# aim-uofa/GenPercept

Hardware: NVIDIA H100
Metric: images/sec at 768x768 depth (higher is better)
Workload: dtype f16

## Files before the change

genpercept_b200/csrc/builder.cu:

```cuda
#include <algorithm>
#include <cmath>
#include <cstring>

#include <cstdlib>

#include "engine.h"
#include "fattn.h"
#include "fattn512.h"

namespace gp {

constexpr size_t kFusedAttnMinBytes = size_t(2) << 30;

size_t Arena::alloc(size_t bytes) {
  bytes = (bytes + 1023) & ~size_t(1023);
  if (bytes == 0) bytes = 1024;
  for (size_t i = 0; i < blks_.size(); ++i) {
    if (blks_[i].free && blks_[i].size >= bytes) {
      if (blks_[i].size > bytes) {
        Blk rest{blks_[i].off + bytes, blks_[i].size - bytes, true};
        blks_[i].size = bytes;
        blks_.insert(blks_.begin() + i + 1, rest);
      }
      blks_[i].free = false;
// ... 130 lines not shown
  *mt = ts.mt;
}

static void check_cuda(cudaError_t e, const std::string& what) {
  if (e != cudaSuccess) throw GpError(GP_ERR_CUDA, what + ": " + cudaGetErrorString(e));
}
static void finalize_or_throw(IgemmParams* p, const std::string& name) {
  const char* err = igemm_finalize(p);
  if (err) throw GpError(GP_ERR_INVALID, name + ": " + err);
}

static bool gn_fusable(const ConvArgs& a, bool split) {
  const char* on = std::getenv("GP_GN_FUSE");
  const bool off = on == nullptr || on[0] == '0';
  if (off || split || a.mode != 0 || a.ks != 3 || a.srcs.size() != 1 || a.sc.size() > 1) return false;
  const T4& s = a.srcs[0];
  if ((s.W % 128) || (s.C % 64) || (!a.sc.empty() && (a.sc[0].C % 64))) return false;
  const int Cout = a.cout_valid > 0 ? a.cout_valid : a.out.C;
  if (!a.out_f32 && (Cout != a.out.C || (Cout % 64))) return false;
  if (a.flags & IG_GEGLU) return false;
  return true;
}

void Builder::conv(const std::string& name, const ConvArgs& a) {
  GP_REQUIRE(!a.srcs.empty() && a.w != nullptr, name + ": bad conv args");
  const bool gn_fused = a.gn != nullptr && gn_fusable(a, split_);
  if (a.gn != nullptr && !gn_fused) {
    int ctot = 0;
    for (auto& s : a.srcs) ctot += s.C;
    T4 tmp = alloc(a.srcs[0].N, a.srcs[0].H, a.srcs[0].W, ctot);
// ... 23 lines not shown
  for (auto& s : a.sc) bytes += (double)s.bytes();
  if (a.res1) bytes += (double)a.res1->bytes();
  if (a.res2) bytes += (double)a.res2->bytes();
  if (!a.out_f32) GP_REQUIRE(a.out.N == N && a.out.H == Ho && a.out.W == Wo, name + ": output shape mismatch");
  const bool tokens_mode = (a.ks == 1 && a.mode == 0 && a.sc.empty() && a.srcs.size() == 1 && !a.out_f32);
  const long long work_px = tokens_mode ? (long long)N * H * W
                                        : (long long)(a.mode == 3 ? W : Wo) * (a.mode == 3 ? H : Ho) * N * (a.mode == 3 ? 4 : 1);
  int bn_pre = choose_bn(Cout, a.force_bn);
  int mt_pre = (bn_pre <= 64 && work_px >= 256LL * num_sms) ? 2 : 1;
  if (!a.force_bn && !(a.flags & IG_GEGLU) && !gn_fused) {
    const double k_elems = flops / (2.0 * N * Ho * Wo * (double)Cout) * (a.mode == 3 ? 4.0 / 9.0 : 1.0);
    tile_shape_for(Cout, k_elems, tokens_mode, N * (a.mode == 3 ? 4 : 1), (a.mode == 3) ? W : Wo, (a.mode == 3) ? H : Ho, num_sms,
                   &bn_pre, &mt_pre);
  }
  const bool staged = !a.out_f32 && !(a.flags & IG_GEGLU) && Cout == a.out.C && (Cout % 64) == 0 && (bn_pre % 64) == 0;
  const bool patch_eligible = gn_fused || (staged && a.mode == 0 && a.ks == 3 && a.srcs.size() == 1 && a.sc.empty() &&
                                           work_px >= 128LL * num_sms && (W % 128) == 0 && !split_);
  if (patch_eligible) {
    bn_pre = (bn_pre == 128 && mt_pre == 1 && staged) ? 128 : 64;
    mt_pre = 1;
  }
  bool emit_stats = a.want_stats && staged && Cout <= 512 && !split_;
  if (emit_stats && tokens_mode && ((long long)H * W) % (128 * mt_pre) != 0) emit_stats = false;
  size_t stats_off = 0;
  const size_t stats_bytes = (size_t)N * num_sms * Cout * 2 * sizeof(float);
  if (emit_stats) {
    GP_REQUIRE(stats.find(a.out.off) == stats.end(), name + ": output already has statistics");
    stats_off = arena_.alloc(stats_bytes);
    stats[a.out.off] = StatsInfo{stats_off, num_sms, Cout};
  }
  if (measuring_) return;

  IgemmParams p;
  std::memset(&p, 0, sizeof(p));
  p.flags = a.flags | (bf16_ ? IG_BF16 : 0) | (a.out_f32 ? IG_OUT_F32_NCHW : 0);
  p.bias = a.w->bias;
  p.res1 = a.res1 ? ptr(*a.res1) : nullptr;
  p.res2 = a.res2 ? ptr(*a.res2) : nullptr;
  p.out = a.out_f32 ? (void*)a.out_f32 : ptr(a.out);
  p.Cout = Cout;
  p.BN = bn_pre;
  p.Z1 = 1; p.Z0 = 1;
  p.out_sy = p.out_sx = 1;
  const bool tokens = tokens_mode;
// ... 161 lines not shown
    p.tmPatch2 = p.tmPatch;
    if (!a.sc.empty()) {
      const T4& x = a.sc[0];
      p.kc_sc = ceil_div(x.C, 64);
      check_cuda(make_tmap_a(&p.tmPatch2, ptr(x), x.C, W, H, N, x.C, (long long)W * x.C, (long long)H * W * x.C,
                             p.TW + 2, p.TH + 2, bf16_), name + ": tmap patch (shortcut)");
    }
    if (gn_fused) {
      p.gn_ss = gn_ss;
      p.gn_C = s0.C;
      p.gn_silu = a.gn_silu ? 1 : 0;
    }
  }
  if (emit_stats) {
    p.stats = reinterpret_cast<float*>(raw_ptr(stats_off));
    p.stats_slots = num_sms;
    p.stats_hw = tokens ? H * W : 0;
  }
  finalize_or_throw(&p, name);
  GP_REQUIRE(p.MT == mt_pre && p.BN == bn_pre, name + ": tile pre-selection disagrees with the plan");
  const int ncls = p.cls_from_z0 ? p.Z0 : 1;
  for (int c = 0; c < ncls; ++c)
    GP_REQUIRE(p.nkb[c] * 64 == a.w->ktot, name + ": packed K (" + std::to_string(a.w->ktot) + ") != planned K (" +
                                              std::to_string(p.nkb[c] * 64) + ")");
  GP_REQUIRE(a.w->rows >= Cout || a.w->rows == Cout, name + ": packed rows < Cout");
  if (emit_stats) {
    float* sp = p.stats;
    push(name, 2, flops, bytes, [p, sp, stats_bytes](cudaStream_t s) {
      cudaError_t e = cudaMemsetAsync(sp, 0, stats_bytes, s);
      if (e != cudaSuccess) return e;
      return igemm_launch(p, s);
// ... 416 lines not shown
```

genpercept_b200/csrc/igemm.cu:

```cuda
#include "igemm.h"

#include <cstring>

#include "igemm_common.cuh"
#include "launch.h"

namespace gp {

namespace {

template <bool BF16, int BN, int MB>
__device__ __forceinline__ void tap_consumer(const IgemmParams& p, uint8_t* smem, int stage_bytes, int a_bytes, float* accs,
                                             uint64_t* full_bar, uint64_t* empty_bar, uint64_t* tfull_bar, uint64_t* tempty_bar,
                                             int wc, int lane) {
  float d[MB][BN / 2];
  int stage = 0;
  uint32_t phase = 0, acc_phase = 0;
  for (int tile = blockIdx.x; tile < p.total_tiles; tile += gridDim.x) {
    const TileCoord t = decode_tile(p, tile);
    const int cls = p.cls_from_z0 ? t.z0 : 0;
    const int nkb = p.nkb[cls] * p.npass;
    int held = -1;
    for (int kb = 0; kb < nkb; ++kb) {
      mbar_wait(&full_bar[stage], phase, 3);
// ... 72 lines not shown
      mbar_init(&full_bar[i], 2);
      mbar_init(&empty_bar[i], 4);
    }
    mbar_init(tfull_bar, 128);
    mbar_init(tempty_bar, kEpiWarps * 32);
    for (int i = 0; i < kEpiWarps; ++i) mbar_init(&res_bar[i], 1);
    fence_barrier_init();
  }
  __syncthreads();

  if (warp < 8) {
    setmaxnreg_inc<kWorkerRegs>();
    if (warp >= kConsumerWarp0) {
      run_tap_consumer<BF16>(p, smem, stage_bytes, a_bytes, accs, full_bar, empty_bar, tfull_bar, tempty_bar, warp - kConsumerWarp0, lane);
    } else {
      if (p.tma_store) run_epilogue_staged<BF16, false>(p, stg_base, sacc, sbias, tfull_bar, tempty_bar, res_bar, accs, warp, lane);
      else run_epilogue_direct<BF16>(p, sbias, tfull_bar, tempty_bar, accs, warp, lane);
    }
    return;
  }
  setmaxnreg_dec<kProducerRegs>();

  if (warp == 8) {
    const bool leader = elect_one();
    int stage = 0;
    uint32_t phase = 0;
    for (int tile = blockIdx.x; tile < p.total_tiles; tile += gridDim.x) {
      const TileCoord t = decode_tile(p, tile);
      const int cls = p.cls_from_z0 ? t.z0 : 0;
      const int a_n = t.z1 * p.a_n_z1 + t.z0 * p.a_n_z0;
      const int a_k0 = t.z0 * p.a_k_z0;
// ... 120 lines not shown
  p->tiles_x = (p->gridW + p->TW - 1) / p->TW;
  p->tiles_y = (p->gridH + p->TH - 1) / p->TH;
  p->n_tiles_n = (p->Cout + p->BN - 1) / p->BN;
  const int ncls = p->cls_from_z0 ? p->Z0 : 1;
  if (ncls > kMaxClasses) return "too many classes";
  for (int c = 0; c < ncls; ++c) {
    if (p->nseg[c] < 1 || p->nseg[c] > kMaxSegs) return "bad segment count";
    int n = 0;
    for (int s = 0; s < p->nseg[c]; ++s) n += p->seg[c][s].nchunks;
    p->nkb[c] = n;
    if (n < 1) return "empty K loop";
  }
  long long total = (long long)p->n_tiles_n * p->tiles_x * p->tiles_y * p->Z0 * p->Z1;
  if (total > 0x7fffffffLL) return "too many tiles";
  p->total_tiles = (int)total;
  const int stats_bytes = p->stats ? 4 * p->Cout * 2 * (int)sizeof(float) : 0;
  if (p->tma_store && ((p->Cout % 64) || (p->BN % 64) || (p->flags & (IG_OUT_F32_NCHW | IG_GEGLU)) || p->out_z0 != 0))
    return "staged epilogue needs Cout % 64 == 0, BN % 64 == 0, plain 16-bit NHWC output, no GEGLU";
  if (p->stats && (!p->tma_store || p->Cout > 512)) return "statistics need the staged epilogue and Cout <= 512";
  p->acc_half = (p->patch && p->BN == 128) ? 1 : 0;
  if (p->acc_half && (!p->tma_store || p->MT != 1))
    return "patch mode at BN = 128 needs the staged epilogue and MT = 1";
  p->acc_pitch = p->acc_half ? 64 : (p->BN + 31) & ~31;
  const int fixed = (p->tma_store ? kEpiWarps * 4096 * (p->out_lo ? 2 : 1) : 0) + acc_tile_bytes(*p) + 3072 + stats_bytes;
  const int ring_unit = p->patch ? p->BN * 128 : kABytes * p->MT + p->BN * 128;
  if (p->patch) {
    if (p->TW != 128 || p->TH != p->MT || p->Z0 != 1 || p->Z1 < 1 || p->nseg[0] != 9 + (p->kc_sc > 0 ? 1 : 0) || p->kc_count < 1 ||
        p->nkb[0] != 9 * p->kc_count + p->kc_sc || p->npass != 1 || p->gridW % 128 || p->gridH % p->TH)
      return "patch mode needs TW = 128, TH = MT, full tiles and a single-source 3x3 tap table (+ shortcut chunks)";
    if (p->gn_ss && p->gn_C != p->kc_count * 64) return "patch mode: GroupNorm channels must equal the source's";
    p->a_slot_bytes = ((p->TW + 2) * (p->TH + 2) * 128 + 1023) & ~1023;
  }
  const int avail = kMaxSmem - 1024 - fixed - (p->patch ? 2 * p->a_slot_bytes : 0);
  int st = avail / ring_unit;
  p->bias_slots = kBiasSlots;
  p->bias_all = 0;
  if (p->n_tiles_n > 1 && p->n_tiles_n * p->BN + 32 <= 4096) {
    const int extra = (p->n_tiles_n * p->BN + 32 - kBiasSlots) * (int)sizeof(float);
    if ((avail - extra) / ring_unit == st) {
      p->bias_all = 1;
      p->bias_slots = p->n_tiles_n * p->BN + 32;
    }
  }
  if (st > 8) st = 8;
  if (st < 2) return "tile too large for shared memory";
  p->stages = st;
  return nullptr;
// ... 9 lines not shown
    cudaError_t e = cudaFuncSetAttribute(igemm_kernel<false>, cudaFuncAttributeMaxDynamicSharedMemorySize, kMaxSmem);
    if (e != cudaSuccess) return e;
    e = cudaFuncSetAttribute(igemm_kernel<true>, cudaFuncAttributeMaxDynamicSharedMemorySize, kMaxSmem);
    if (e != cudaSuccess) return e;
    cudaDeviceGetAttribute(&sms[dev], cudaDevAttrMultiProcessorCount, dev);
    attr_set[dev] = true;
  }
  g_num_sms = sms[dev];
  return cudaSuccess;
}

cudaError_t igemm_launch(const IgemmParams& p, cudaStream_t stream) {
  cudaError_t ie = igemm_init();
  if (ie != cudaSuccess) return ie;
  if (p.total_tiles <= 0) return cudaSuccess;
  if (p.stats && p.stats_slots < (p.total_tiles < g_num_sms ? p.total_tiles : g_num_sms)) return cudaErrorInvalidValue;
  const int grid = p.total_tiles < g_num_sms ? p.total_tiles : g_num_sms;
  const size_t smem = kMaxSmem;
  if (p.patch) return igemm_patch_launch(p, grid, stream);
  if (p.flags & IG_BF16) {
    launch(igemm_kernel<true>, grid, kRoleThreads, smem, stream, p);
  } else {
    launch(igemm_kernel<false>, grid, kRoleThreads, smem, stream, p);
  }
  return cudaGetLastError();
}

}
```

genpercept_b200/csrc/igemm.h:

```cpp
#pragma once
#include <cuda.h>
#include <cuda_runtime.h>
#include <stdint.h>

namespace gp {

constexpr int kMaxSegs = 20;
constexpr int kMaxClasses = 4;
constexpr int kBM = 128;
constexpr int kBK = 64;

struct IgemmSeg {
  int8_t map;
  int8_t dy, dx;
  uint16_t nchunks;
};

enum IgemmFlags : int {
  IG_RELU = 1,
  IG_OUT_F32_NCHW = 2,
  IG_AFFINE_CLAMP01 = 4,
  IG_BF16 = 8,
  IG_GEGLU = 16,
};
// ... 30 lines not shown
  const float* bias;
  const void* res1;
  const void* res2;
  int flags;
  int stages;
  int total_tiles;
  float* stats;
  int stats_slots;
  int stats_hw;
  int tma_store;
  CUtensorMap tmOut[kMaxClasses];
  int res_tma;
  int bias_slots;
  int bias_all;
  int acc_pitch;
  int acc_half;
  CUtensorMap tmRes[kMaxClasses];
  int patch;
  int kc_count;
  int kc_sc;
  int a_slot_bytes;
  CUtensorMap tmPatch;
  CUtensorMap tmPatch2;
  const float* gn_ss;
  int gn_C;
  int gn_silu;
};

cudaError_t igemm_patch_launch(const IgemmParams& p, int grid, cudaStream_t stream);

cudaError_t make_tmap_a(CUtensorMap* m, const void* base, int C, int W, int H, int N, long long sW,
// ... 8 lines not shown
```

genpercept_b200/csrc/igemm_common.cuh:

```cuda
#pragma once
#include <cuda_bf16.h>
#include <cuda_fp16.h>

#include "igemm.h"
#include "ptx.cuh"

namespace gp {
namespace {

constexpr int kABytes = kBM * kBK * 2;
constexpr int kMaxSmem = 227 * 1024;
constexpr int kEpiWarps = 4;
constexpr int kConsumerWarp0 = 4;
constexpr int kRoleThreads = 384;
constexpr int kProducerRegs = 40;
constexpr int kWorkerRegs = 232;
static_assert(128 * kProducerRegs + 256 * kWorkerRegs <= 65536, "register file of one SM");

struct TileCoord {
  int n_tile, tx, ty, z0, z1;
};

__device__ __forceinline__ TileCoord decode_tile(const IgemmParams& p, int tile) {
  TileCoord t;
// ... 63 lines not shown
  for (int q = 0; q < N / 4; ++q) {
    const float4 v = *reinterpret_cast<const float4*>(rp + (acc_chunk((c >> 2) + q, row) << 2));
    r[4 * q] = __float_as_uint(v.x); r[4 * q + 1] = __float_as_uint(v.y);
    r[4 * q + 2] = __float_as_uint(v.z); r[4 * q + 3] = __float_as_uint(v.w);
  }
}

template <int BN, bool BF16>
__device__ __forceinline__ void wgmma_ss(float (&d)[BN / 2], uint64_t a, uint64_t b, uint32_t acc) {
  if constexpr (BN == 16) wgmma_ss_n16<BF16>(d, a, b, acc);
  else if constexpr (BN == 32) wgmma_ss_n32<BF16>(d, a, b, acc);
  else if constexpr (BN == 64) wgmma_ss_n64<BF16>(d, a, b, acc);
  else wgmma_ss_n128<BF16>(d, a, b, acc);
}

template <int BN, int MB, int J0 = 0, int NJ = BN / 8>
__device__ __forceinline__ void acc_store(float* accs, int pitch, float (&d)[MB][BN / 2], int wc, int lane) {
#pragma unroll
  for (int mb = 0; mb < MB; ++mb) {
    reg_fence(d[mb]);
#pragma unroll
    for (int j = J0; j < J0 + NJ; ++j)
#pragma unroll
      for (int hh = 0; hh < 2; ++hh) {
        const int row = 64 * mb + 16 * wc + (lane >> 2) + 8 * hh, col = 8 * (j - J0) + 2 * (lane & 3);
        *reinterpret_cast<float2*>(accs + (size_t)row * pitch + (acc_chunk(col >> 2, row) << 2) + (col & 3)) =
            make_float2(d[mb][4 * j + 2 * hh], d[mb][4 * j + 2 * hh + 1]);
      }
  }
}

__device__ __forceinline__ float gelu_erf(float g) {
  const float z = fabsf(g) * 0.70710678118654752f;
  float t;
  asm("rcp.approx.ftz.f32 %0, %1;" : "=f"(t) : "f"(fmaf(0.3275911f, z, 1.f)));
  float e;
  asm("ex2.approx.ftz.f32 %0, %1;" : "=f"(e) : "f"(z * z * -1.4426950408889634f));
  float q = fmaf(1.061405429f, t, -1.453152027f);
  q = fmaf(q, t, 1.421413741f);
  q = fmaf(q, t, -0.284496736f);
// ... 25 lines not shown
}

template <bool BF16, bool SPLIT, int RES>
__device__ __forceinline__ void epilogue_staged(const IgemmParams& p, uint8_t* stg_base, float* sacc, float* sbias, uint64_t* tfull_bar,
                                                uint64_t* tempty_bar, uint64_t* res_bar, const float* accs, int warp, int lane) {
  const int wq = warp;
  uint8_t* stg = stg_base + warp * 4096;
  const uint32_t stg_addr = smem_u32(stg);
  const uint32_t my_row = stg_addr + lane * 128;
  constexpr bool split = SPLIT;
  const uint32_t my_row_lo = my_row + kEpiWarps * 4096;
  const int sw = lane & 7;
  uint32_t acc_phase = 0, res_phase = 0;
  const bool relu = (p.flags & IG_RELU) != 0;
  const bool do_stats = p.stats != nullptr;
  const bool halves = p.acc_half != 0;
  const int etid = threadIdx.x;
  int cur_img = -1;
  int cur_nt = -1;
  auto flush_stats = [&](int img) {
    epi_sync();
    float* dst = p.stats + ((long long)img * p.stats_slots + blockIdx.x) * p.Cout * 2;
    for (int i = etid; i < 2 * p.Cout; i += kEpiWarps * 32) {
      const float tot = (sacc[i] + sacc[2 * p.Cout + i]) + (sacc[4 * p.Cout + i] + sacc[6 * p.Cout + i]);
      dst[i] = tot;
      sacc[i] = 0.f; sacc[2 * p.Cout + i] = 0.f; sacc[4 * p.Cout + i] = 0.f; sacc[6 * p.Cout + i] = 0.f;
    }
    epi_sync();
  };
  if (do_stats) {
    for (int i = etid; i < 8 * p.Cout; i += kEpiWarps * 32) sacc[i] = 0.f;
// ... 26 lines not shown
        if (cur_img >= 0) flush_stats(cur_img);
        cur_img = img;
      }
    }
    for (int h = 0; h < p.MT; ++h) {
      const int r0 = h * 128 + wq * 32;
      const int row = r0 + lane;
      const int ti = row >> p.tw_shift, tj = row & (p.TW - 1);
      const int gy = t.ty * p.TH + ti, gx = t.tx * p.TW + tj;
      const bool valid = gy < p.gridH && gx < p.gridW;
      const int oy = gy * p.out_sy + p.cls_py[cls], ox = gx * p.out_sx + p.cls_px[cls];
      const long long pix_off = t.z1 * p.out_z1 + (long long)oy * p.out_row_stride + (long long)ox * p.out_pix_stride;
      const int sx = t.tx * p.TW + (r0 & (p.TW - 1)), sy = t.ty * p.TH + (r0 >> p.tw_shift);
      for (int c0 = 0; c0 < p.BN; c0 += 64) {
        const int n0 = n_base + c0;
        if (n0 >= p.Cout) {
          if (!halves) break;
          mbar_wait(tfull_bar, acc_phase, 4);
          mbar_arrive(tempty_bar);
          acc_phase ^= 1;
          continue;
        }
        if (lane == 0) tma_store_wait_read0();
        __syncwarp();
        uint4 rt[8];
        if constexpr (RES == 1) {
          if (lane == 0) {
            mbar_expect_tx(&res_bar[warp], 4096);
            tma_load_4d(stg, &p.tmRes[cls], &res_bar[warp], n0, sx, sy, t.z1);
          }
          mbar_wait(&res_bar[warp], res_phase, 7);
          res_phase ^= 1;
#pragma unroll
          for (int i = 0; i < 8; ++i)
            asm volatile("ld.shared.v4.b32 {%0, %1, %2, %3}, [%4];"
                         : "=r"(rt[i].x), "=r"(rt[i].y), "=r"(rt[i].z), "=r"(rt[i].w)
                         : "r"(my_row + ((i ^ sw) << 4)));
// ... 10 lines not shown
          uint4 r1[4], r2[4];
          const bool has1 = RES == 1 || (RES == 2 && valid && p.res1 != nullptr), has2 = RES == 2 && valid && p.res2 != nullptr;
          if constexpr (RES == 1) {
#pragma unroll
            for (int q = 0; q < 4; ++q) r1[q] = rt[sub * 4 + q];
          } else if (has1) {
            const uint4* rp = reinterpret_cast<const uint4*>(reinterpret_cast<const uint16_t*>(p.res1) + off);
#pragma unroll
            for (int q = 0; q < 4; ++q) r1[q] = rp[q];
          }
          if (has2) {
            const uint4* rp = reinterpret_cast<const uint4*>(reinterpret_cast<const uint16_t*>(p.res2) + off);
#pragma unroll
            for (int q = 0; q < 4; ++q) r2[q] = rp[q];
          }
          if (halves) {
            if (sub == 0) {
              mbar_wait(tfull_bar, acc_phase, 4);
              acc_ld<32>(accs, p.acc_pitch, row, 0, rh[0]);
              acc_ld<32>(accs, p.acc_pitch, row, 32, rh[1]);
              mbar_arrive(tempty_bar);
              acc_phase ^= 1;
            }
          } else {
            if (!waited) {
              mbar_wait(tfull_bar, acc_phase, 4);
              waited = true;
            }
            acc_ld<32>(accs, p.acc_pitch, row, c0 + sub * 32, rh[sub]);
          }
          const uint32_t (&r)[32] = rh[sub];
          float v[32];
#pragma unroll
          for (int q = 0; q < 32; ++q) v[q] = __uint_as_float(r[q]) + bz[q];
          if (has1) {
#pragma unroll
            for (int q = 0; q < 4; ++q) add8<BF16>(&v[q * 8], r1[q]);
          }
          if (has2) {
#pragma unroll
            for (int q = 0; q < 4; ++q) add8<BF16>(&v[q * 8], r2[q]);
          }
          if (split) {
            if (has1) {
              const uint4* rp = reinterpret_cast<const uint4*>(reinterpret_cast<const uint16_t*>(p.res1) + off + p.out_lo);
// ... 42 lines not shown
        if (do_stats) {
          const uint32_t col = stg_addr + (lane & 3) * 4;
          const int chunk = lane >> 2;
#pragma unroll 8
          for (int rr = 0; rr < 32; ++rr) {
            uint32_t w;
            asm volatile("ld.shared.b32 %0, [%1];" : "=r"(w) : "r"(col + rr * 128 + ((chunk ^ (rr & 7)) << 4)));
            const float a = cvt16<BF16>((uint16_t)(w & 0xFFFF)), b = cvt16<BF16>((uint16_t)(w >> 16));
            s0 += a; q0 += a * a; s1 += b; q1 += b * b;
          }
          float* d = sacc + ((size_t)wq * p.Cout + n0 + 2 * lane) * 2;
          d[0] += s0; d[1] += q0; d[2] += s1; d[3] += q1;
        }
      }
    }
    if (!halves) {
      if (!waited) {
        mbar_wait(tfull_bar, acc_phase, 4);
      }
      mbar_arrive(tempty_bar);
      acc_phase ^= 1;
    }
  }
  if (lane == 0) tma_store_wait_read0();
  if (do_stats && cur_img >= 0) flush_stats(cur_img);
}


template <bool BF16, bool LEAN>
__device__ __forceinline__ void run_epilogue_staged(const IgemmParams& p, uint8_t* stg_base, float* sacc, float* sbias, uint64_t* tfull_bar,
                                                    uint64_t* tempty_bar, uint64_t* res_bar, const float* accs, int warp, int lane) {
  const int rm = p.res_tma ? 1 : ((p.res1 != nullptr || p.res2 != nullptr) ? 2 : 0);
  if constexpr (!LEAN) {
    if (p.out_lo != 0) {
      if (rm == 2) epilogue_staged<BF16, true, 2>(p, stg_base, sacc, sbias, tfull_bar, tempty_bar, res_bar, accs, warp, lane);
      else epilogue_staged<BF16, true, 0>(p, stg_base, sacc, sbias, tfull_bar, tempty_bar, res_bar, accs, warp, lane);
      return;
    }
  }
  if (rm == 1) epilogue_staged<BF16, false, 1>(p, stg_base, sacc, sbias, tfull_bar, tempty_bar, res_bar, accs, warp, lane);
  else if (rm == 2) epilogue_staged<BF16, false, 2>(p, stg_base, sacc, sbias, tfull_bar, tempty_bar, res_bar, accs, warp, lane);
  else epilogue_staged<BF16, false, 0>(p, stg_base, sacc, sbias, tfull_bar, tempty_bar, res_bar, accs, warp, lane);
}

template <bool BF16, bool LEAN>
__device__ __forceinline__ void epilogue_direct(const IgemmParams& p, float* sbias, uint64_t* tfull_bar, uint64_t* tempty_bar,
                                                const float* accs, int warp, int lane) {
  const int wq = warp;
  uint32_t acc_phase = 0;
  const bool f32out = !LEAN && (p.flags & IG_OUT_F32_NCHW) != 0;
  const bool relu = !LEAN && (p.flags & IG_RELU) != 0;
  const bool aff = !LEAN && (p.flags & IG_AFFINE_CLAMP01) != 0;
  const bool geglu = LEAN || (p.flags & IG_GEGLU) != 0;
// ... 150 lines not shown
```

genpercept_b200/csrc/igemm_patch.cu:

```cuda
#include "igemm_common.cuh"
#include "launch.h"

namespace gp {

namespace {

constexpr int kPW = kBM + 2;
constexpr int kPP = kPW;

__device__ __forceinline__ float silu_tanh(float x) {
  const float h = 0.5f * x;
  float t;
  asm("tanh.approx.f32 %0, %1;" : "=f"(t) : "f"(h));
  return fmaf(h, t, h);
}
__device__ __forceinline__ uint32_t silu_pair_f16(float ha, float hb) {
  const __half2 h2 = __floats2half2_rn(ha, hb);
  uint32_t hi = *reinterpret_cast<const uint32_t*>(&h2), ti;
  asm("tanh.approx.f16x2 %0, %1;" : "=r"(ti) : "r"(hi));
  const float2 t = __half22float2(*reinterpret_cast<const __half2*>(&ti));
  const __half2 y = __floats2half2_rn(fmaf(ha, t.x, ha), fmaf(hb, t.y, hb));
  return *reinterpret_cast<const uint32_t*>(&y);
}

template <bool BF16>
__device__ __forceinline__ void transform_patch(const IgemmParams& p, uint32_t slot_addr, const TileCoord& t, int kc, int tt) {
  const int cpos = tt & 7;
  const int rbase = tt >> 3;
  const int jlog = cpos ^ (rbase & 7);
  const bool do_silu = p.gn_silu != 0;
  const int prows = (p.TH + 2) * kPP;
  const int x0 = t.tx * p.TW - 1, y0 = t.ty * p.TH - 1;
  float sc[8], sh[8];
  const float4* sp = reinterpret_cast<const float4*>(p.gn_ss + (long long)t.z1 * p.gn_C * 2 + (kc * kBK + jlog * 8) * 2);
  const float pre = (do_silu && !BF16) ? 0.5f : 1.f;
#pragma unroll
  for (int e = 0; e < 4; ++e) {
    const float4 a = __ldg(sp + e);
    sc[2 * e] = a.x * pre; sh[2 * e] = a.y * pre; sc[2 * e + 1] = a.z * pre; sh[2 * e + 1] = a.w * pre;
  }
  const uint32_t base = slot_addr + cpos * 16;
// ... 18 lines not shown
      for (int e = 0; e < 4; ++e) {
        float a = fmaf(cvt16<BF16>((uint16_t)(w[u][e] & 0xFFFF)), sc[2 * e], sh[2 * e]);
        float b = fmaf(cvt16<BF16>((uint16_t)(w[u][e] >> 16)), sc[2 * e + 1], sh[2 * e + 1]);
        if (BF16) {
          if (do_silu) { a = silu_tanh(a); b = silu_tanh(b); }
          w[u][e] = pack16<BF16>(a, b);
        } else {
          w[u][e] = do_silu ? silu_pair_f16(a, b) : pack16<BF16>(a, b);
        }
      }
      asm volatile("st.shared.v4.b32 [%0], {%1, %2, %3, %4};" ::"r"(base + (r + 16 * u) * 128), "r"(w[u][0]),
                   "r"(w[u][1]), "r"(w[u][2]), "r"(w[u][3]) : "memory");
    }
  }
  fence_proxy_async_shared();
  asm volatile("bar.sync 2, 128;" ::: "memory");
}

template <bool BF16, bool XFORM, int BN, int MB>
__device__ __forceinline__ void patch_consumer(const IgemmParams& p, uint8_t* smem, uint8_t* sB, float* accs, uint64_t* a_full,
                                               uint64_t* a_empty, uint64_t* b_full, uint64_t* b_empty, uint64_t* tfull_bar,
                                               uint64_t* tempty_bar, int wc, int lane) {
  float d[MB][BN / 2];
  const int b_bytes = BN * 128;
  const int kc_all = p.kc_count + p.kc_sc;
  int slot = 0, stage = 0;
  uint32_t a_phase = 0, b_phase = 0, acc_phase = 0;
  auto row_off = [&](int mb, int dy, int dx) { return ((dy + 1 + (mb >> 1)) * kPP + dx + 1 + (mb & 1) * 64) * 128; };
  for (int tile = blockIdx.x; tile < p.total_tiles; tile += gridDim.x) {
    const TileCoord t = decode_tile(p, tile);
    int held_stage = -1;
    int held_slot = -1;
    for (int kc = 0; kc < kc_all; ++kc) {
      const bool main = kc < p.kc_count;
      mbar_wait(&a_full[slot], a_phase, 3);
      const uint32_t patch = smem_u32(smem + slot * p.a_slot_bytes);
      if constexpr (XFORM) {
        if (main) transform_patch<BF16>(p, patch, t, kc, wc * 32 + lane);
      }
      const int ntap = main ? 9 : 1;
      for (int tap = 0; tap < ntap; ++tap) {
        const int dy = main ? p.seg[0][tap].dy : 0, dx = main ? p.seg[0][tap].dx : 0;
        mbar_wait(&b_full[stage], b_phase, 6);
        const uint64_t b_desc = make_sw128_kmajor_desc(smem_u32(sB + stage * b_bytes));
#pragma unroll
        for (int mb = 0; mb < MB; ++mb) reg_fence(d[mb]);
        wgmma_fence();
#pragma unroll
        for (int mb = 0; mb < MB; ++mb) {
          const uint64_t a_desc = make_sw128_kmajor_desc(patch + row_off(mb, dy, dx));
#pragma unroll
          for (int k = 0; k < kBK / 16; ++k) wgmma_ss<BN, BF16>(d[mb], a_desc + 2 * k, b_desc + 2 * k, (kc | tap | k) ? 1u : 0u);
        }
// ... 3 lines not shown
        for (int mb = 0; mb < MB; ++mb) reg_fence(d[mb]);
        if (held_stage >= 0) {
          __syncwarp();
          if (lane == 0) {
            mbar_arrive(&b_empty[held_stage]);
            if (held_slot >= 0) mbar_arrive(&a_empty[held_slot]);
          }
          held_slot = -1;
        }
        held_stage = stage;
        if (++stage == p.stages) { stage = 0; b_phase ^= 1; }
      }
      held_slot = slot;
      if (++slot == 2) { slot = 0; a_phase ^= 1; }
    }
    wgmma_wait<0>();
#pragma unroll
    for (int mb = 0; mb < MB; ++mb) reg_fence(d[mb]);
    __syncwarp();
    if (lane == 0) {
      mbar_arrive(&b_empty[held_stage]);
      mbar_arrive(&a_empty[held_slot]);
    }
    if constexpr (BN == 128) {
      mbar_wait(tempty_bar, acc_phase ^ 1, 2);
      acc_store<BN, MB, 0, 8>(accs, p.acc_pitch, d, wc, lane);
      mbar_arrive(tfull_bar);
      acc_phase ^= 1;
      mbar_wait(tempty_bar, acc_phase ^ 1, 2);
      acc_store<BN, MB, 8, 8>(accs, p.acc_pitch, d, wc, lane);
      mbar_arrive(tfull_bar);
      acc_phase ^= 1;
    } else {
      mbar_wait(tempty_bar, acc_phase ^ 1, 2);
      acc_store<BN, MB>(accs, p.acc_pitch, d, wc, lane);
      mbar_arrive(tfull_bar);
      acc_phase ^= 1;
    }
  }
}

template <bool BF16, bool XFORM>
__global__ void __launch_bounds__(kRoleThreads, 1) igemm_patch_kernel(const __grid_constant__ IgemmParams p) {
  extern __shared__ uint8_t smem_raw[];
  uint8_t* smem = reinterpret_cast<uint8_t*>((reinterpret_cast<uintptr_t>(smem_raw) + 1023) & ~uintptr_t(1023));
  const int b_bytes = p.BN * 128;
  const int stages = p.stages;
  uint8_t* sB = smem + 2 * p.a_slot_bytes;
  uint8_t* stg_base = sB + stages * b_bytes;
  float* accs = reinterpret_cast<float*>(stg_base + (p.tma_store ? kEpiWarps * 4096 : 0));
  uint64_t* a_full = reinterpret_cast<uint64_t*>(accs + 128 * p.MT * p.acc_pitch);
  uint64_t* a_empty = a_full + 2;
  uint64_t* b_full = a_empty + 2;
  uint64_t* b_empty = b_full + stages;
  uint64_t* tfull_bar = b_empty + stages;
  uint64_t* tempty_bar = tfull_bar + 1;
  uint64_t* res_bar = tempty_bar + 1;
  float* sbias = reinterpret_cast<float*>((reinterpret_cast<uintptr_t>(res_bar + kEpiWarps) + 15) & ~uintptr_t(15));
  float* sacc = sbias + p.bias_slots;

  const int warp = uniform_warp_id();
  const int lane = threadIdx.x & 31;
  const int kc_all = p.kc_count + p.kc_sc;

  if (threadIdx.x == 0) {
    tma_prefetch_desc(&p.tmPatch);
    tma_prefetch_desc(&p.tmPatch2);
    tma_prefetch_desc(&p.tmB);
    for (int i = 0; i < 2; ++i) {
      mbar_init(&a_full[i], 1);
      mbar_init(&a_empty[i], 4);
    }
    for (int i = 0; i < stages; ++i) { mbar_init(&b_full[i], 1); mbar_init(&b_empty[i], 4); }
    mbar_init(tfull_bar, 128);
    mbar_init(tempty_bar, kEpiWarps * 32);
    for (int i = 0; i < kEpiWarps; ++i) mbar_init(&res_bar[i], 1);
    fence_barrier_init();
  }
  __syncthreads();

  if (warp < 8) {
    setmaxnreg_inc<kWorkerRegs>();
    if (warp < kEpiWarps) {
      if (p.tma_store) run_epilogue_staged<BF16, true>(p, stg_base, sacc, sbias, tfull_bar, tempty_bar, res_bar, accs, warp, lane);
      else epilogue_direct<BF16, false>(p, sbias, tfull_bar, tempty_bar, accs, warp, lane);
    } else {
      const int wc = warp - kConsumerWarp0;
#define GP_PATCH(BN_, MB_) patch_consumer<BF16, XFORM, BN_, MB_>(p, smem, sB, accs, a_full, a_empty, b_full, b_empty, tfull_bar, tempty_bar, wc, lane)
      if (p.MT == 2) {
        if (p.BN == 16) GP_PATCH(16, 4); else if (p.BN == 32) GP_PATCH(32, 4); else GP_PATCH(64, 4);
      } else {
        if (p.BN == 16) GP_PATCH(16, 2); else if (p.BN == 32) GP_PATCH(32, 2); else if (p.BN == 64) GP_PATCH(64, 2); else GP_PATCH(128, 2);
      }
#undef GP_PATCH
    }
    return;
  }
  setmaxnreg_dec<kProducerRegs>();
  if (warp == 8) {
    const bool leader = elect_one();
    int slot = 0;
    uint32_t phase = 0;
    for (int tile = blockIdx.x; tile < p.total_tiles; tile += gridDim.x) {
      const TileCoord t = decode_tile(p, tile);
      const int x0 = t.tx * p.TW - 1, y0 = t.ty * p.TH - 1;
      for (int kc = 0; kc < kc_all; ++kc) {
        const bool main = kc < p.kc_count;
        mbar_wait(&a_empty[slot], phase ^ 1, 1);
        if (leader) {
          mbar_expect_tx(&a_full[slot], (uint32_t)((p.TH + 2) * kPW * 128));
// ... 61 lines not shown
```

Measured before the change: 44.95.

## Run two consumer warpgroups ping-pong in patch conv with in-register epilogue

The patch-mode implicit GEMM kernel drops its dedicated epilogue warps and shared fp32 accumulator staging. Instead, two 4-warp consumer groups each take alternate tiles and write their own epilogue (bias, residual via TMA, relu, stats, TMA store) straight from registers. Named barriers hand the MMA turn between groups, so one group's epilogue overlaps the other's mainloop. Patch mode is restricted to MT=1 rows, and stats slots double so each warpgroup gets its own partial sums.

```diff
diff --git a/genpercept_b200/csrc/builder.cu b/genpercept_b200/csrc/builder.cu
--- a/genpercept_b200/csrc/builder.cu
+++ b/genpercept_b200/csrc/builder.cu
@@ -168,6 +168,7 @@
   const char* on = std::getenv("GP_GN_FUSE");
   const bool off = on == nullptr || on[0] == '0';
   if (off || split || a.mode != 0 || a.ks != 3 || a.srcs.size() != 1 || a.sc.size() > 1) return false;
+  if (a.res2 != nullptr || (a.out_f32 && a.res1 != nullptr)) return false;
   const T4& s = a.srcs[0];
   if ((s.W % 128) || (s.C % 64) || (!a.sc.empty() && (a.sc[0].C % 64))) return false;
   const int Cout = a.cout_valid > 0 ? a.cout_valid : a.out.C;
@@ -221,7 +222,7 @@
                    &bn_pre, &mt_pre);
   }
   const bool staged = !a.out_f32 && !(a.flags & IG_GEGLU) && Cout == a.out.C && (Cout % 64) == 0 && (bn_pre % 64) == 0;
-  const bool patch_eligible = gn_fused || (staged && a.mode == 0 && a.ks == 3 && a.srcs.size() == 1 && a.sc.empty() &&
+  const bool patch_eligible = gn_fused || (staged && a.mode == 0 && a.ks == 3 && a.srcs.size() == 1 && a.sc.empty() && !a.res2 &&
                                            work_px >= 128LL * num_sms && (W % 128) == 0 && !split_);
   if (patch_eligible) {
     bn_pre = (bn_pre == 128 && mt_pre == 1 && staged) ? 128 : 64;
@@ -230,11 +231,12 @@
   bool emit_stats = a.want_stats && staged && Cout <= 512 && !split_;
   if (emit_stats && tokens_mode && ((long long)H * W) % (128 * mt_pre) != 0) emit_stats = false;
   size_t stats_off = 0;
-  const size_t stats_bytes = (size_t)N * num_sms * Cout * 2 * sizeof(float);
+  const int stats_slots = (patch_eligible ? 2 : 1) * num_sms;
+  const size_t stats_bytes = (size_t)N * stats_slots * Cout * 2 * sizeof(float);
   if (emit_stats) {
     GP_REQUIRE(stats.find(a.out.off) == stats.end(), name + ": output already has statistics");
     stats_off = arena_.alloc(stats_bytes);
-    stats[a.out.off] = StatsInfo{stats_off, num_sms, Cout};
+    stats[a.out.off] = StatsInfo{stats_off, stats_slots, Cout};
   }
   if (measuring_) return;
 
@@ -426,7 +428,7 @@
   }
   if (emit_stats) {
     p.stats = reinterpret_cast<float*>(raw_ptr(stats_off));
-    p.stats_slots = num_sms;
+    p.stats_slots = stats_slots;
     p.stats_hw = tokens ? H * W : 0;
   }
   finalize_or_throw(&p, name);
diff --git a/genpercept_b200/csrc/igemm.cu b/genpercept_b200/csrc/igemm.cu
--- a/genpercept_b200/csrc/igemm.cu
+++ b/genpercept_b200/csrc/igemm.cu
@@ -110,7 +110,7 @@
     if (warp >= kConsumerWarp0) {
       run_tap_consumer<BF16>(p, smem, stage_bytes, a_bytes, accs, full_bar, empty_bar, tfull_bar, tempty_bar, warp - kConsumerWarp0, lane);
     } else {
-      if (p.tma_store) run_epilogue_staged<BF16, false>(p, stg_base, sacc, sbias, tfull_bar, tempty_bar, res_bar, accs, warp, lane);
+      if (p.tma_store) run_epilogue_staged<BF16>(p, stg_base, sacc, sbias, tfull_bar, tempty_bar, res_bar, accs, warp, lane);
       else run_epilogue_direct<BF16>(p, sbias, tfull_bar, tempty_bar, accs, warp, lane);
     }
     return;
@@ -261,23 +261,27 @@
   long long total = (long long)p->n_tiles_n * p->tiles_x * p->tiles_y * p->Z0 * p->Z1;
   if (total > 0x7fffffffLL) return "too many tiles";
   p->total_tiles = (int)total;
-  const int stats_bytes = p->stats ? 4 * p->Cout * 2 * (int)sizeof(float) : 0;
   if (p->tma_store && ((p->Cout % 64) || (p->BN % 64) || (p->flags & (IG_OUT_F32_NCHW | IG_GEGLU)) || p->out_z0 != 0))
     return "staged epilogue needs Cout % 64 == 0, BN % 64 == 0, plain 16-bit NHWC output, no GEGLU";
   if (p->stats && (!p->tma_store || p->Cout > 512)) return "statistics need the staged epilogue and Cout <= 512";
-  p->acc_half = (p->patch && p->BN == 128) ? 1 : 0;
-  if (p->acc_half && (!p->tma_store || p->MT != 1))
-    return "patch mode at BN = 128 needs the staged epilogue and MT = 1";
-  p->acc_pitch = p->acc_half ? 64 : (p->BN + 31) & ~31;
-  const int fixed = (p->tma_store ? kEpiWarps * 4096 * (p->out_lo ? 2 : 1) : 0) + acc_tile_bytes(*p) + 3072 + stats_bytes;
-  const int ring_unit = p->patch ? p->BN * 128 : kABytes * p->MT + p->BN * 128;
+  p->acc_pitch = (p->BN + 31) & ~31;
+  int fixed;
   if (p->patch) {
-    if (p->TW != 128 || p->TH != p->MT || p->Z0 != 1 || p->Z1 < 1 || p->nseg[0] != 9 + (p->kc_sc > 0 ? 1 : 0) || p->kc_count < 1 ||
-        p->nkb[0] != 9 * p->kc_count + p->kc_sc || p->npass != 1 || p->gridW % 128 || p->gridH % p->TH)
-      return "patch mode needs TW = 128, TH = MT, full tiles and a single-source 3x3 tap table (+ shortcut chunks)";
+    if (p->TW != 128 || p->TH != 1 || p->MT != 1 || p->Z0 != 1 || p->Z1 < 1 || p->nseg[0] != 9 + (p->kc_sc > 0 ? 1 : 0) ||
+        p->kc_count < 1 || p->nkb[0] != 9 * p->kc_count + p->kc_sc || p->npass != 1 || p->gridW % 128)
+      return "patch mode needs one full 128-pixel image row per tile and a single-source 3x3 tap table (+ shortcut chunks)";
+    if (p->BN != 64 && p->BN != 128) return "patch mode needs BN = 64 or 128";
+    if (p->tma_store ? (p->res2 != nullptr || (p->res1 != nullptr && !p->res_tma))
+                     : (!(p->flags & IG_OUT_F32_NCHW) || p->BN != 64 || p->res1 != nullptr || p->res2 != nullptr))
+      return "patch mode writes through the staged epilogue (residual by TMA only) or an fp32 map at BN = 64";
     if (p->gn_ss && p->gn_C != p->kc_count * 64) return "patch mode: GroupNorm channels must equal the source's";
     p->a_slot_bytes = ((p->TW + 2) * (p->TH + 2) * 128 + 1023) & ~1023;
-  }
+    fixed = (p->tma_store ? 2 * kBM * 64 * 2 : 0) + 3072 + (p->stats ? 2 * 4 * p->Cout * 2 * (int)sizeof(float) : 0);
+  } else {
+    fixed = (p->tma_store ? kEpiWarps * 4096 * (p->out_lo ? 2 : 1) : 0) + acc_tile_bytes(*p) + 3072 +
+            (p->stats ? 4 * p->Cout * 2 * (int)sizeof(float) : 0);
+  }
+  const int ring_unit = p->patch ? p->BN * 128 : kABytes * p->MT + p->BN * 128;
   const int avail = kMaxSmem - 1024 - fixed - (p->patch ? 2 * p->a_slot_bytes : 0);
   int st = avail / ring_unit;
   p->bias_slots = kBiasSlots;
@@ -317,8 +321,8 @@
   cudaError_t ie = igemm_init();
   if (ie != cudaSuccess) return ie;
   if (p.total_tiles <= 0) return cudaSuccess;
-  if (p.stats && p.stats_slots < (p.total_tiles < g_num_sms ? p.total_tiles : g_num_sms)) return cudaErrorInvalidValue;
   const int grid = p.total_tiles < g_num_sms ? p.total_tiles : g_num_sms;
+  if (p.stats && p.stats_slots < (p.patch ? 2 : 1) * grid) return cudaErrorInvalidValue;
   const size_t smem = kMaxSmem;
   if (p.patch) return igemm_patch_launch(p, grid, stream);
   if (p.flags & IG_BF16) {
diff --git a/genpercept_b200/csrc/igemm.h b/genpercept_b200/csrc/igemm.h
--- a/genpercept_b200/csrc/igemm.h
+++ b/genpercept_b200/csrc/igemm.h
@@ -68,7 +68,6 @@
   int bias_slots;
   int bias_all;
   int acc_pitch;
-  int acc_half;
   CUtensorMap tmRes[kMaxClasses];
   int patch;
   int kc_count;
diff --git a/genpercept_b200/csrc/igemm_common.cuh b/genpercept_b200/csrc/igemm_common.cuh
--- a/genpercept_b200/csrc/igemm_common.cuh
+++ b/genpercept_b200/csrc/igemm_common.cuh
@@ -101,16 +101,16 @@
   else wgmma_ss_n128<BF16>(d, a, b, acc);
 }
 
-template <int BN, int MB, int J0 = 0, int NJ = BN / 8>
+template <int BN, int MB>
 __device__ __forceinline__ void acc_store(float* accs, int pitch, float (&d)[MB][BN / 2], int wc, int lane) {
 #pragma unroll
   for (int mb = 0; mb < MB; ++mb) {
     reg_fence(d[mb]);
 #pragma unroll
-    for (int j = J0; j < J0 + NJ; ++j)
+    for (int j = 0; j < BN / 8; ++j)
 #pragma unroll
       for (int hh = 0; hh < 2; ++hh) {
-        const int row = 64 * mb + 16 * wc + (lane >> 2) + 8 * hh, col = 8 * (j - J0) + 2 * (lane & 3);
+        const int row = 64 * mb + 16 * wc + (lane >> 2) + 8 * hh, col = 8 * j + 2 * (lane & 3);
         *reinterpret_cast<float2*>(accs + (size_t)row * pitch + (acc_chunk(col >> 2, row) << 2) + (col & 3)) =
             make_float2(d[mb][4 * j + 2 * hh], d[mb][4 * j + 2 * hh + 1]);
       }
@@ -166,7 +166,6 @@
   uint32_t acc_phase = 0, res_phase = 0;
   const bool relu = (p.flags & IG_RELU) != 0;
   const bool do_stats = p.stats != nullptr;
-  const bool halves = p.acc_half != 0;
   const int etid = threadIdx.x;
   int cur_img = -1;
   int cur_nt = -1;
@@ -223,13 +222,7 @@
       const int sx = t.tx * p.TW + (r0 & (p.TW - 1)), sy = t.ty * p.TH + (r0 >> p.tw_shift);
       for (int c0 = 0; c0 < p.BN; c0 += 64) {
         const int n0 = n_base + c0;
-        if (n0 >= p.Cout) {
-          if (!halves) break;
-          mbar_wait(tfull_bar, acc_phase, 4);
-          mbar_arrive(tempty_bar);
-          acc_phase ^= 1;
-          continue;
-        }
+        if (n0 >= p.Cout) break;
         if (lane == 0) tma_store_wait_read0();
         __syncwarp();
         uint4 rt[8];
@@ -270,21 +263,11 @@
 #pragma unroll
             for (int q = 0; q < 4; ++q) r2[q] = rp[q];
           }
-          if (halves) {
-            if (sub == 0) {
-              mbar_wait(tfull_bar, acc_phase, 4);
-              acc_ld<32>(accs, p.acc_pitch, row, 0, rh[0]);
-              acc_ld<32>(accs, p.acc_pitch, row, 32, rh[1]);
-              mbar_arrive(tempty_bar);
-              acc_phase ^= 1;
-            }
-          } else {
-            if (!waited) {
-              mbar_wait(tfull_bar, acc_phase, 4);
-              waited = true;
-            }
-            acc_ld<32>(accs, p.acc_pitch, row, c0 + sub * 32, rh[sub]);
-          }
+          if (!waited) {
+            mbar_wait(tfull_bar, acc_phase, 4);
+            waited = true;
+          }
+          acc_ld<32>(accs, p.acc_pitch, row, c0 + sub * 32, rh[sub]);
           const uint32_t (&r)[32] = rh[sub];
           float v[32];
 #pragma unroll
@@ -357,29 +340,25 @@
         }
       }
     }
-    if (!halves) {
-      if (!waited) {
-        mbar_wait(tfull_bar, acc_phase, 4);
-      }
-      mbar_arrive(tempty_bar);
-      acc_phase ^= 1;
-    }
+    if (!waited) {
+      mbar_wait(tfull_bar, acc_phase, 4);
+    }
+    mbar_arrive(tempty_bar);
+    acc_phase ^= 1;
   }
   if (lane == 0) tma_store_wait_read0();
   if (do_stats && cur_img >= 0) flush_stats(cur_img);
 }
 
 
-template <bool BF16, bool LEAN>
+template <bool BF16>
 __device__ __forceinline__ void run_epilogue_staged(const IgemmParams& p, uint8_t* stg_base, float* sacc, float* sbias, uint64_t* tfull_bar,
                                                     uint64_t* tempty_bar, uint64_t* res_bar, const float* accs, int warp, int lane) {
   const int rm = p.res_tma ? 1 : ((p.res1 != nullptr || p.res2 != nullptr) ? 2 : 0);
-  if constexpr (!LEAN) {
-    if (p.out_lo != 0) {
-      if (rm == 2) epilogue_staged<BF16, true, 2>(p, stg_base, sacc, sbias, tfull_bar, tempty_bar, res_bar, accs, warp, lane);
-      else epilogue_staged<BF16, true, 0>(p, stg_base, sacc, sbias, tfull_bar, tempty_bar, res_bar, accs, warp, lane);
-      return;
-    }
+  if (p.out_lo != 0) {
+    if (rm == 2) epilogue_staged<BF16, true, 2>(p, stg_base, sacc, sbias, tfull_bar, tempty_bar, res_bar, accs, warp, lane);
+    else epilogue_staged<BF16, true, 0>(p, stg_base, sacc, sbias, tfull_bar, tempty_bar, res_bar, accs, warp, lane);
+    return;
   }
   if (rm == 1) epilogue_staged<BF16, false, 1>(p, stg_base, sacc, sbias, tfull_bar, tempty_bar, res_bar, accs, warp, lane);
   else if (rm == 2) epilogue_staged<BF16, false, 2>(p, stg_base, sacc, sbias, tfull_bar, tempty_bar, res_bar, accs, warp, lane);
diff --git a/genpercept_b200/csrc/igemm_patch.cu b/genpercept_b200/csrc/igemm_patch.cu
--- a/genpercept_b200/csrc/igemm_patch.cu
+++ b/genpercept_b200/csrc/igemm_patch.cu
@@ -7,6 +7,12 @@
 
 constexpr int kPW = kBM + 2;
 constexpr int kPP = kPW;
+constexpr int kTurnBar0 = 1;
+constexpr int kWgBar0 = 3;
+
+__device__ __forceinline__ void wg_sync(int wg) { asm volatile("bar.sync %0, 128;" ::"r"(kWgBar0 + wg) : "memory"); }
+__device__ __forceinline__ void turn_wait(int wg) { asm volatile("bar.sync %0, 256;" ::"r"(kTurnBar0 + wg) : "memory"); }
+__device__ __forceinline__ void turn_pass(int wg) { asm volatile("bar.arrive %0, 256;" ::"r"(kTurnBar0 + (wg ^ 1)) : "memory"); }
 
 __device__ __forceinline__ float silu_tanh(float x) {
   const float h = 0.5f * x;
@@ -24,7 +30,7 @@
 }
 
 template <bool BF16>
-__device__ __forceinline__ void transform_patch(const IgemmParams& p, uint32_t slot_addr, const TileCoord& t, int kc, int tt) {
+__device__ __forceinline__ void transform_patch(const IgemmParams& p, uint32_t slot_addr, const TileCoord& t, int kc, int tt, int wg) {
   const int cpos = tt & 7;
   const int rbase = tt >> 3;
   const int jlog = cpos ^ (rbase & 7);
@@ -73,29 +79,69 @@
     }
   }
   fence_proxy_async_shared();
-  asm volatile("bar.sync 2, 128;" ::: "memory");
-}
-
-template <bool BF16, bool XFORM, int BN, int MB>
-__device__ __forceinline__ void patch_consumer(const IgemmParams& p, uint8_t* smem, uint8_t* sB, float* accs, uint64_t* a_full,
-                                               uint64_t* a_empty, uint64_t* b_full, uint64_t* b_empty, uint64_t* tfull_bar,
-                                               uint64_t* tempty_bar, int wc, int lane) {
+  wg_sync(wg);
+}
+
+template <bool BF16, bool XFORM, int OUT, int BN>
+__device__ __forceinline__ void patch_consumer(const IgemmParams& p, uint8_t* smem, uint8_t* sB, uint8_t* stg, float* sacc,
+                                               uint64_t* a_full, uint64_t* a_empty, uint64_t* b_full, uint64_t* b_empty,
+                                               uint64_t* res_bar, int wg, int wc, int lane) {
+  constexpr int MB = 2;
+  constexpr int kParts = 4;
   float d[MB][BN / 2];
   const int b_bytes = BN * 128;
   const int kc_all = p.kc_count + p.kc_sc;
-  int slot = 0, stage = 0;
-  uint32_t a_phase = 0, b_phase = 0, acc_phase = 0;
-  auto row_off = [&](int mb, int dy, int dx) { return ((dy + 1 + (mb >> 1)) * kPP + dx + 1 + (mb & 1) * 64) * 128; };
-  for (int tile = blockIdx.x; tile < p.total_tiles; tile += gridDim.x) {
+  const int nb = 9 * p.kc_count + p.kc_sc;
+  const int wt = wc * 32 + lane;
+  const bool issuer = wt == 0;
+  const uint32_t stg_addr = smem_u32(stg);
+  const bool do_stats = OUT < 2 && p.stats != nullptr;
+  const bool relu = (p.flags & IG_RELU) != 0;
+  float* my_sacc = sacc + wg * kParts * p.Cout * 2;
+  uint32_t res_phase = 0;
+  int cur_img = -1;
+  auto flush_stats = [&](int img) {
+    wg_sync(wg);
+    float* dst = p.stats + ((long long)img * p.stats_slots + 2 * blockIdx.x + wg) * p.Cout * 2;
+    for (int i = wt; i < 2 * p.Cout; i += 128) {
+      dst[i] = (my_sacc[i] + my_sacc[2 * p.Cout + i]) + (my_sacc[4 * p.Cout + i] + my_sacc[6 * p.Cout + i]);
+#pragma unroll
+      for (int k = 0; k < kParts; ++k) my_sacc[2 * k * p.Cout + i] = 0.f;
+    }
+    wg_sync(wg);
+  };
+  if (do_stats) {
+    for (int i = wt; i < kParts * 2 * p.Cout; i += 128) my_sacc[i] = 0.f;
+    wg_sync(wg);
+  }
+  auto row_off = [&](int mb, int dy, int dx) { return ((dy + 1) * kPP + dx + 1 + mb * 64) * 128; };
+  int q = wg;
+  for (int tile = blockIdx.x + wg * gridDim.x; tile < p.total_tiles; tile += 2 * gridDim.x, q += 2) {
     const TileCoord t = decode_tile(p, tile);
+    const int n_base = t.n_tile * BN;
+    const int sx = t.tx * kBM, sy = t.ty;
+    auto load_res = [&](int g) {
+      mbar_expect_tx(res_bar, 128 * 128);
+      for (int r = 0; r < 4; ++r) tma_load_4d(stg + r * 4096, &p.tmRes[0], res_bar, n_base + 64 * g, sx + 32 * r, sy, t.z1);
+    };
+    if constexpr (OUT == 1) {
+      if (issuer) {
+        tma_store_wait_read0();
+        load_res(0);
+      }
+    }
+    const int c0 = q * kc_all, b0 = q * nb;
+    int slot = c0 & 1, stage = b0 % p.stages;
+    uint32_t a_phase = (c0 >> 1) & 1, b_phase = (b0 / p.stages) & 1;
     int held_stage = -1;
     int held_slot = -1;
+    if (tile != (int)blockIdx.x) turn_wait(wg);
     for (int kc = 0; kc < kc_all; ++kc) {
       const bool main = kc < p.kc_count;
       mbar_wait(&a_full[slot], a_phase, 3);
       const uint32_t patch = smem_u32(smem + slot * p.a_slot_bytes);
       if constexpr (XFORM) {
-        if (main) transform_patch<BF16>(p, patch, t, kc, wc * 32 + lane);
+        if (main) transform_patch<BF16>(p, patch, t, kc, wt, wg);
       }
       const int ntap = main ? 9 : 1;
       for (int tap = 0; tap < ntap; ++tap) {
@@ -129,6 +175,7 @@
       held_slot = slot;
       if (++slot == 2) { slot = 0; a_phase ^= 1; }
     }
+    if (tile + (int)gridDim.x < p.total_tiles) turn_pass(wg);
     wgmma_wait<0>();
 #pragma unroll
     for (int mb = 0; mb < MB; ++mb) reg_fence(d[mb]);
@@ -137,22 +184,102 @@
       mbar_arrive(&b_empty[held_stage]);
       mbar_arrive(&a_empty[held_slot]);
     }
-    if constexpr (BN == 128) {
-      mbar_wait(tempty_bar, acc_phase ^ 1, 2);
-      acc_store<BN, MB, 0, 8>(accs, p.acc_pitch, d, wc, lane);
-      mbar_arrive(tfull_bar);
-      acc_phase ^= 1;
-      mbar_wait(tempty_bar, acc_phase ^ 1, 2);
-      acc_store<BN, MB, 8, 8>(accs, p.acc_pitch, d, wc, lane);
-      mbar_arrive(tfull_bar);
-      acc_phase ^= 1;
+
+    if constexpr (OUT == 2) {
+      const bool aff = (p.flags & IG_AFFINE_CLAMP01) != 0;
+      float* o = reinterpret_cast<float*>(p.out);
+#pragma unroll
+      for (int j = 0; j < BN / 8; ++j) {
+#pragma unroll
+        for (int e = 0; e < 2; ++e) {
+          const int n = n_base + 8 * j + 2 * (lane & 3) + e;
+          if (n >= p.Cout) continue;
+          const float bz = p.bias != nullptr ? __ldg(p.bias + n) : 0.f;
+          float* on = o + (((long long)t.z1 * p.Cout + n) * p.outH + sy) * p.outW + sx;
+#pragma unroll
+          for (int mb = 0; mb < MB; ++mb)
+#pragma unroll
+            for (int hh = 0; hh < 2; ++hh) {
+              float x = d[mb][4 * j + 2 * hh + e] + bz;
+              if (relu) x = fmaxf(x, 0.f);
+              if (aff) x = fminf(fmaxf((x + 1.f) * 0.5f, 0.f), 1.f);
+              on[64 * mb + 16 * wc + (lane >> 2) + 8 * hh] = x;
+            }
+        }
+      }
     } else {
-      mbar_wait(tempty_bar, acc_phase ^ 1, 2);
-      acc_store<BN, MB>(accs, p.acc_pitch, d, wc, lane);
-      mbar_arrive(tfull_bar);
-      acc_phase ^= 1;
-    }
-  }
+      if (do_stats && t.z1 != cur_img) {
+        if (cur_img >= 0) flush_stats(cur_img);
+        cur_img = t.z1;
+      }
+      const int r7 = lane >> 2;
+#pragma unroll
+      for (int g = 0; g < BN / 64; ++g) {
+        if (n_base + 64 * g >= p.Cout) break;
+        if (g > 0) {
+          if (issuer) {
+            tma_store_wait_read0();
+            if constexpr (OUT == 1) load_res(g);
+          }
+        }
+        if constexpr (OUT == 1) {
+          mbar_wait(res_bar, res_phase, 7);
+          res_phase ^= 1;
+        } else {
+          if (issuer && g == 0) tma_store_wait_read0();
+          wg_sync(wg);
+        }
+#pragma unroll
+        for (int jj = 0; jj < 8; ++jj) {
+          const int j = 8 * g + jj;
+          const int n = n_base + 8 * j + 2 * (lane & 3);
+          const float b0v = p.bias != nullptr ? __ldg(p.bias + n) : 0.f;
+          const float b1v = p.bias != nullptr ? __ldg(p.bias + n + 1) : 0.f;
+          const uint32_t cbase = stg_addr + ((jj ^ r7) << 4) + (lane & 3) * 4;
+#pragma unroll
+          for (int mb = 0; mb < MB; ++mb)
+#pragma unroll
+            for (int hh = 0; hh < 2; ++hh) {
+              const uint32_t a = cbase + (64 * mb + 16 * wc + (lane >> 2) + 8 * hh) * 128;
+              float v0 = d[mb][4 * j + 2 * hh] + b0v, v1 = d[mb][4 * j + 2 * hh + 1] + b1v;
+              if constexpr (OUT == 1) {
+                uint32_t w;
+                asm volatile("ld.shared.b32 %0, [%1];" : "=r"(w) : "r"(a));
+                v0 += cvt16<BF16>((uint16_t)(w & 0xFFFF));
+                v1 += cvt16<BF16>((uint16_t)(w >> 16));
+              }
+              if (relu) { v0 = fmaxf(v0, 0.f); v1 = fmaxf(v1, 0.f); }
+              asm volatile("st.shared.b32 [%0], %1;" ::"r"(a), "r"(pack16<BF16>(v0, v1)) : "memory");
+            }
+        }
+        fence_proxy_async_shared();
+        wg_sync(wg);
+        if (issuer) {
+          for (int r = 0; r < 4; ++r) tma_store_4d(&p.tmOut[0], stg_addr + r * 4096, n_base + 64 * g, sx + 32 * r, sy, t.z1);
+          tma_store_commit();
+        }
+        if (do_stats) {
+          const int cp = lane, n = n_base + 64 * g + 2 * cp;
+          const uint32_t col = stg_addr + (cp & 3) * 4;
+          const int chunk = cp >> 2;
+          float s0 = 0.f, s1 = 0.f, q0 = 0.f, q1 = 0.f;
+#pragma unroll 8
+          for (int rr = 0; rr < 32; ++rr) {
+            const int row = 32 * wc + rr;
+            uint32_t w;
+            asm volatile("ld.shared.b32 %0, [%1];" : "=r"(w) : "r"(col + row * 128 + ((chunk ^ (row & 7)) << 4)));
+            const float a = cvt16<BF16>((uint16_t)(w & 0xFFFF)), b = cvt16<BF16>((uint16_t)(w >> 16));
+            s0 += a; q0 += a * a; s1 += b; q1 += b * b;
+          }
+          float* dp = my_sacc + ((size_t)wc * p.Cout + n) * 2;
+          dp[0] += s0; dp[1] += q0; dp[2] += s1; dp[3] += q1;
+          wg_sync(wg);
+        }
+      }
+    }
+  }
+  if (OUT < 2 && issuer) tma_store_wait_read0();
+  if (do_stats && cur_img >= 0) flush_stats(cur_img);
 }
 
 template <bool BF16, bool XFORM>
@@ -162,17 +289,14 @@
   const int b_bytes = p.BN * 128;
   const int stages = p.stages;
   uint8_t* sB = smem + 2 * p.a_slot_bytes;
-  uint8_t* stg_base = sB + stages * b_bytes;
-  float* accs = reinterpret_cast<float*>(stg_base + (p.tma_store ? kEpiWarps * 4096 : 0));
-  uint64_t* a_full = reinterpret_cast<uint64_t*>(accs + 128 * p.MT * p.acc_pitch);
+  uint8_t* stg0 = sB + stages * b_bytes;
+  const int stg_bytes = p.tma_store ? kBM * 64 * 2 : 0;
+  uint64_t* a_full = reinterpret_cast<uint64_t*>(stg0 + 2 * stg_bytes);
   uint64_t* a_empty = a_full + 2;
   uint64_t* b_full = a_empty + 2;
   uint64_t* b_empty = b_full + stages;
-  uint64_t* tfull_bar = b_empty + stages;
-  uint64_t* tempty_bar = tfull_bar + 1;
-  uint64_t* res_bar = tempty_bar + 1;
-  float* sbias = reinterpret_cast<float*>((reinterpret_cast<uintptr_t>(res_bar + kEpiWarps) + 15) & ~uintptr_t(15));
-  float* sacc = sbias + p.bias_slots;
+  uint64_t* res_bar = b_empty + stages;
+  float* sacc = reinterpret_cast<float*>((reinterpret_cast<uintptr_t>(res_bar + 2) + 15) & ~uintptr_t(15));
 
   const int warp = uniform_warp_id();
   const int lane = threadIdx.x & 31;
@@ -185,30 +309,23 @@
     for (int i = 0; i < 2; ++i) {
       mbar_init(&a_full[i], 1);
       mbar_init(&a_empty[i], 4);
+      mbar_init(&res_bar[i], 1);
     }
     for (int i = 0; i < stages; ++i) { mbar_init(&b_full[i], 1); mbar_init(&b_empty[i], 4); }
-    mbar_init(tfull_bar, 128);
-    mbar_init(tempty_bar, kEpiWarps * 32);
-    for (int i = 0; i < kEpiWarps; ++i) mbar_init(&res_bar[i], 1);
     fence_barrier_init();
   }
   __syncthreads();
 
   if (warp < 8) {
     setmaxnreg_inc<kWorkerRegs>();
-    if (warp < kEpiWarps) {
-      if (p.tma_store) run_epilogue_staged<BF16, true>(p, stg_base, sacc, sbias, tfull_bar, tempty_bar, res_bar, accs, warp, lane);
-      else epilogue_direct<BF16, false>(p, sbias, tfull_bar, tempty_bar, accs, warp, lane);
-    } else {
-      const int wc = warp - kConsumerWarp0;
-#define GP_PATCH(BN_, MB_) patch_consumer<BF16, XFORM, BN_, MB_>(p, smem, sB, accs, a_full, a_empty, b_full, b_empty, tfull_bar, tempty_bar, wc, lane)
-      if (p.MT == 2) {
-        if (p.BN == 16) GP_PATCH(16, 4); else if (p.BN == 32) GP_PATCH(32, 4); else GP_PATCH(64, 4);
-      } else {
-        if (p.BN == 16) GP_PATCH(16, 2); else if (p.BN == 32) GP_PATCH(32, 2); else if (p.BN == 64) GP_PATCH(64, 2); else GP_PATCH(128, 2);
-      }
+    const int wg = warp >> 2, wc = warp & 3;
+    uint8_t* stg = stg0 + wg * stg_bytes;
+#define GP_PATCH(OUT_, BN_) \
+  patch_consumer<BF16, XFORM, OUT_, BN_>(p, smem, sB, stg, sacc, a_full, a_empty, b_full, b_empty, &res_bar[wg], wg, wc, lane)
+    if (!p.tma_store) GP_PATCH(2, 64);
+    else if (p.res_tma) { if (p.BN == 128) GP_PATCH(1, 128); else GP_PATCH(1, 64); }
+    else { if (p.BN == 128) GP_PATCH(0, 128); else GP_PATCH(0, 64); }
 #undef GP_PATCH
-    }
     return;
   }
   setmaxnreg_dec<kProducerRegs>();
```

After: 45.88, median of 6. 1.02x the previous value.
